# rasmusab/bayes.js

Hardware: AMD Instinct MI355X
Metric: posterior draws/sec (= param-updates/sec) (higher is better)
Workload: dtype f64

## Files before the change

bayes.js_amd/csrc/amwg_kernel.h:

```cpp
#pragma once
#if !defined(__HIPCC_RTC__)
#include <hip/hip_runtime.h>
#endif

#include "amwg_div.h"
#include "amwg_ld.h"
#include "amwg_philox.h"
#include "amwg_types.h"

namespace amwg {

struct LdsLayout {
  uint32_t data, state, pls, cnt, tot, cc, adapt, pl, idx, perm, total, stride, logpls, bc, xw;
};
__host__ __device__ inline LdsLayout lds_layout(size_t data_bytes, int P, int CPB, int max_top, int n_named, bool multi = false) {
  LdsLayout L;
  uint32_t o = 0;
  L.stride = (uint32_t)P | 1u;
  L.data = o;  o += (uint32_t)((data_bytes + 15) & ~(size_t)15);
  L.state = o; o += L.stride * CPB * 8;
  L.pls = o;   o += L.stride * CPB * 8;
  L.cnt = o;   o += L.stride * CPB * 8;
  L.tot = o;   o += (L.stride * CPB * 4 + 15) & ~15u;
  L.cc = o;    o += (uint32_t)P * sizeof(CompConst);
// ... 374 lines not shown
      "s_cselect_b64 %[m], %[OA], %[EA]\n\t"
      "s_branch 4f\n"
      "3:\n\t"
      "s_bitcmp1_b32 %[p], 0\n\t"
      "s_cselect_b64 %[m], %[OB], %[EB]\n"
      "4:\n\t"
      "s_bfe_u32 %[tmp], %[p], 0x60001\n\t"
      "s_lshr_b64 %[rest], %[m], %[tmp]\n\t"
      "s_cmp_lg_u64 %[rest], 0\n\t"
      "s_cbranch_scc1 6f\n\t"
      "s_and_b32 %[tmp], %[p], 1\n\t"
      "s_bitcmp1_b32 %[p], 7\n\t"
      "s_cbranch_scc1 5f\n\t"
      "s_or_b32 %[p], %[tmp], 0x80\n\t"
      "s_branch 2b\n"
      "5:\n\t"
      "s_or_b32 %[p], %[tmp], 0xfe\n\t"
      "s_branch 9f\n"
      "6:\n\t"
      "s_ff1_i32_b64 %[tmp], %[rest]\n\t"
      "s_lshl_b32 %[tmp], %[tmp], 1\n\t"
      "s_add_u32 %[p], %[p], %[tmp]\n\t"
      "s_mov_b32 m0, %[t]\n\t"
      "v_writelane_b32 %[ppv], %[p], m0\n\t"
      "s_add_u32 %[p], %[p], 3\n\t"
      "s_add_u32 %[t], %[t], 1\n\t"
      "s_branch 1b\n"
      "9:\n\t"
      "s_mov_b32 m0, %[km0]"
      : [p] "+s"(p), [t] "+s"(t), [ppv] "+v"(ppv), [m] "=&s"(m), [rest] "=&s"(rest), [tmp] "=&s"(tmp), [km0] "=&s"(keep_m0)
      : [EA] "s"(EA), [OA] "s"(OA), [EB] "s"(EB), [OB] "s"(OB), [top] "s"(top)
      : "scc");
#endif
}

template <int G>
__device__ __forceinline__ int chain_uniform(int v) {
#if defined(__HIP_DEVICE_COMPILE__)
  if constexpr (G >= 64) return __builtin_amdgcn_readfirstlane(v);
#endif
  return v;
}

__device__ __forceinline__ double lane_value(double v, int src) {
#if defined(__HIP_DEVICE_COMPILE__)
  const uint32_t hi = (uint32_t)__builtin_amdgcn_readlane((int)(f64_bits(v) >> 32), src);
  const uint32_t lo = (uint32_t)__builtin_amdgcn_readlane((int)(uint32_t)f64_bits(v), src);
  return bits_f64(((uint64_t)hi << 32) | (uint64_t)lo);
#else
  return v;
#endif
}

constexpr int kErrReplicasNeedOneWave = 1, kErrLaunchTooLong = 2, kErrMirrorOutOfSync = 4, kErrSweepNeedsOrderInRegisters = 8, kErrNoKernelBody = 16;
__device__ __forceinline__ void device_error(const StepArgs &a, int code) {
#if defined(__HIP_DEVICE_COMPILE__)
  if (threadIdx.x == 0) (void)atomicOr(a.ch.error, code);
#endif
}
template <class M, class = void> struct MirrorCheckOf { static constexpr bool value = false; };
template <class M> struct MirrorCheckOf<M, void_of<decltype(M::kMirrorCheck)>> { static constexpr bool value = M::kMirrorCheck; };

template <class Model, int G, int BT = 256, bool GL = false, bool SW = false, bool CT = false>
__device__ __forceinline__ void step_body(const StepArgs &a, unsigned char *smem) {
  constexpr int kPassU = SW ? (CertNeedsRows<Model>::value ? 2 : 4) : (BT >= 1024 ? 4 : 8);
  const int tid = threadIdx.x, nt = blockDim.x;
  constexpr bool kMulti = G > 64;
  if (!kMulti && a.cpb > 0 && nt != 64) { device_error(a, kErrReplicasNeedOneWave); return; }
  if (a.n_steps > 65535) { device_error(a, kErrLaunchTooLong); return; }
  const int CPB = kMulti ? G / 64 : ((a.cpb > 0 && a.cpb < nt / G) ? a.cpb : nt / G);
  const int c_raw = kMulti ? tid / 64 : tid / G;
  const int c_in = c_raw < CPB ? c_raw : CPB - 1, sub = tid % G;
  const int P = a.pl.P;
  const int n_named = a.pl.n_params;
  const LdsLayout L = lds_layout(DataBytesOf<Model, GL>::get(a.d, G, nt), P, CPB, a.pl.max_top, n_named, kMulti);

  const unsigned char *data_lds = smem + L.data;
  double *Sblk = reinterpret_cast<double *>(smem + L.state);
  CompConst *cc = reinterpret_cast<CompConst *>(smem + L.cc);
  uint8_t *adapt = smem + L.adapt;
  int32_t *pl_base = reinterpret_cast<int32_t *>(smem + L.pl), *pl_len = pl_base + n_named, *pl_top = pl_len + n_named, *pl_multidim = pl_top + n_named, *pl_inner = pl_multidim + n_named;
  const bool wide_idx = a.pl.max_top > kByteTop, wide_perm = n_named > kPackedNamed;
  const IndexColumn idx{smem + L.idx + (wide_idx ? 2 * c_in : c_in), CPB, wide_idx};
  const IndexColumn pcol{smem + L.perm + 2 * c_in, CPB, true};
  double *SDme = reinterpret_cast<double *>(smem + L.pls) + (size_t)c_in * L.stride;
  int2 *CNTme = reinterpret_cast<int2 *>(smem + L.cnt) + (size_t)c_in * L.stride;
  uint32_t *TOTme = reinterpret_cast<uint32_t *>(smem + L.tot) + (size_t)c_in * L.stride;
  double *LOGPLSme = reinterpret_cast<double *>(smem + L.logpls) + (size_t)c_in * L.stride;
  int32_t *BCme = reinterpret_cast<int32_t *>(smem + L.bc) + (size_t)c_in * L.stride;
  CrossWave xw{reinterpret_cast<double *>(smem + L.xw), 0};
  typename CacheOf<Model>::type cache = CacheOf<Model>::init();

  Model::stage(smem + L.data, a.d, tid, nt, G);
  for (int p = tid; p < P; p += nt) { cc[p] = a.cc[p]; adapt[p] = a.is_adapting[p]; }
  for (int i = tid; i < 4 * n_named; i += nt) pl_base[i] = a.pl.tab[i];
  for (int i = tid; i < n_named; i += nt) pl_inner[i] = a.pl.tab[n_named + i] / a.pl.tab[2 * n_named + i];

  const int64_t chain_raw = kMulti ? (int64_t)blockIdx.x : (int64_t)blockIdx.x * CPB + c_in;
  const bool live = chain_raw < a.C;
  const int64_t cl = live ? chain_raw : a.C - 1;
  const bool writer = live && sub == 0;
  const bool counter = sub == 0 && c_raw < CPB;
  const int64_t C = a.C;

  double *Sme = Sblk + (size_t)c_in * L.stride;
  for (int p = 0; p < P; ++p) {
    Sme[p] = a.ch.state[p * C + cl];
    SDme[p] = exp_v8(a.ch.prop_log_scale[p * C + cl]);
    CNTme[p] = make_int2(a.ch.acceptance_count[p * C + cl], a.ch.iterations_since_adaption[p * C + cl]);
    TOTme[p] = 0u;
    if constexpr (kMulti) { LOGPLSme[p] = a.ch.prop_log_scale[p * C + cl]; BCme[p] = a.ch.batch_count[p * C + cl]; }
  }
  const StateView S{Sme};
  uint64_t perm = wide_perm ? 0ull : a.ch.perm[cl];
  if (wide_perm)
    for (int k = 0; k < n_named; ++k) pcol.set(k, (int)a.ch.perm16[(int64_t)k * C + cl]);
  typename RngOf<Model, G, GL, SW>::type rng;
  if constexpr (GL) rng.init(a.seed, a.chain_offset + (uint64_t)cl, a.ch.rng_n[cl], tid, reinterpret_cast<double *>(smem + L.data + Model::gl_lds_bytes(a.d.pad, 0)) + (size_t)(tid >> 6) * 256);
  else if constexpr (SW) rng.init(a.seed, a.chain_offset + (uint64_t)cl, a.ch.rng_n[cl], tid, reinterpret_cast<double *>(smem + L.data + Model::window_offset(a.d, nt / 64)) + (size_t)(tid >> 6) * 256);
  else rng.init(a.seed, a.chain_offset + (uint64_t)cl, a.ch.rng_n[cl], tid);
  double lp_curr = a.ch.lp_curr[cl];
  __syncthreads();
  constexpr bool kCert = CT && CertifiedAt<Model, G>::value && !GL && (SW == CertNeedsRows<Model>::value);
  static_assert(kCert == CT, "a certified kernel is instantiated for a model that has no certified value at this lane count");
  constexpr bool kRefOrder = kCert && G > 1 && RefOrderOf<Model>::value;
  auto expression = [&]() -> double {
    if constexpr (kRefOrder) return Model::template reference_order<G>(cache, S, a.mc, a.d, data_lds, sub);
    else if constexpr (!GL) return log_post<Model, G, kPassU>(S, a, data_lds, sub, xw, cache);
    else return 0.0;
  };
  if constexpr (!GL) { if (a.init_lp) lp_curr = expression(); }
  double lpA = lp_curr, epsA = 0.0;
  bool lp_exact = true;
  if constexpr (kCert) { if (!a.init_lp) { epsA = a.ch.lp_eps[cl]; lp_exact = epsA == 0.0; } }
  (void)lpA; (void)epsA; (void)lp_exact;
#if defined(AMWG_AUDIT)
  constexpr bool kAudit = kCert;
#else
  constexpr bool kAudit = false;
#endif
  [[maybe_unused]] double audE = 0.0, aud_max_v = 0.0, aud_max_d = 0.0;
  [[maybe_unused]] uint32_t aud_n = 0u, aud_bad = 0u;
  [[maybe_unused]] auto audit_bin = [&](int which, double ratio) {
#if defined(AMWG_AUDIT)
    if (writer) {
      int b = 0;
      if (ratio > 0.0) { b = (int)((f64_bits(ratio) >> 52) & 0x7ffu) - 1023 + 40; b = b < 1 ? 1 : (b > 63 ? 63 : b); }
      if (!(ratio == ratio)) b = 63;
      (void)atomicAdd(cold_args()->ch.audit_hist + which * 64 + b, 1ull);
    }
#endif
  };
  [[maybe_unused]] auto audit_adversarial_u = [&](double ex, double eta, double u, int parity) -> double {
    if (!(eta < 0x1p-8) || !(ex > 0x1p-900) || !(ex < kInf)) return u;
    const double below = ex * (1.0 - 1.5 * eta), above = ex * (1.0 + 1.5 * eta);
    const double v = ((parity & 1) && above < 1.0) ? above : below;
    return (v > 0.0 && v < 1.0) ? v : u;
  };
  [[maybe_unused]] auto audit_value = [&](double A, double eps, double E) {
    if (eps == eps && eps < kInf && eps > 0.0 && E == E && __builtin_fabs(E) < kInf) {
      const double r = __builtin_fabs(A - E) / eps;
      aud_max_v = (r > aud_max_v || !(r == r)) ? r : aud_max_v;
      audit_bin(0, r);
    }
  };
  [[maybe_unused]] auto audit_difference = [&](double dA, double eta0, double dE, int verdict, double u) {
    if (eta0 == eta0 && eta0 < kInf && eta0 > 0.0 && dE == dE && __builtin_fabs(dE) < kInf) {
      const double r = __builtin_fabs(dA - dE) / eta0;
      aud_max_d = (r > aud_max_d || !(r == r)) ? r : aud_max_d;
      audit_bin(1, r);
    }
    const bool exact_acc = exp_v8(dE) > u;
    ++aud_n;
    if ((verdict > 0 && !exact_acc) || (verdict < 0 && exact_acc)) ++aud_bad;
  };
#if defined(AMWG_X_PHASES)
  uint64_t ph_acc[16];
#pragma unroll
  for (int q = 0; q < 16; ++q) ph_acc[q] = 0;
  uint64_t ph_last = __builtin_readcyclecounter();
#define AMWG_PHASE(i) do { const uint64_t ph_now = __builtin_readcyclecounter(); ph_acc[i] += ph_now - ph_last; ph_last = ph_now; } while (0)
#else
#define AMWG_PHASE(i) do { } while (0)
#endif
  auto set_state = [&](int comp, double v) {
    Sme[comp] = v;
    if constexpr (TracksState<Model>::value) Model::on_set(cache, comp, v, sub, a.d);
  };

  constexpr int D = Model::kDerived;
  const int PR = P + D;
  int64_t row = a.row0;
  int32_t next_rec = (int32_t)a.step0;
  const int P_stepped = a.pl.P_stepped;
  const bool recording = a.draws != nullptr;
  const int n_steps = a.n_steps;

  const int lane64 = tid & 63;
  int ord = lane64;
  (void)ord;
  if (SW && a.pl.max_top > 64) { device_error(a, kErrSweepNeedsOrderInRegisters); return; }
  const bool ord_in_regs = SW ? true : (G >= 64 && a.pl.max_top <= 64);
  constexpr bool kSweep = SW && !GL && LaneReuseOf<Model>::value && G == 64 && !BinaryOf<Model>::value;
  const bool sweep_rt = kSweep && ord_in_regs && a.d.pad > 0;
  if constexpr (kAudit) { if (lp_exact) audE = lp_curr; else audE = expression(); }
  wave_priority(kStepperPriority);
  auto record_draws = [&](int step) {
    if (recording && step == next_rec) {
      double *const draws = cold_args()->draws;
      {
        constexpr int LW = G < 64 ? G : 64;
        if (live && (!kMulti || sub < 64))
          for (int p = sub & (LW - 1); p < P; p += LW) {
#if !defined(AMWG_X_NOREC)
            draws[(row * PR + p) * C + cl] = S(p);
#endif
          }
      }
      if constexpr (D > 0) {
        double dv[D];
        (void)Model::template eval<G, true>(S, a.d, data_lds, sub, dv);
        if (writer)
          for (int q = 0; q < D; ++q) draws[(row * PR + P + q) * C + cl] = dv[q];
      }
      ++row;
      next_rec += cold_args()->thin;
    }
  };
  auto shuffle_named = [&]() {
    for (int i = n_named - 1; i > 0; --i) {
      const int j = (int)__builtin_floor(rng.next() * (double)(i + 1));
      if (wide_perm) { const int ti = pcol.get(i); pcol.set(i, pcol.get(j)); pcol.set(j, ti); }
      else perm = perm_swap(perm, i, j);
    }
  };
  auto adapt_component = [&](int comp, bool accepted, int2 cnt, double batch_size, bool store, bool per_lane = false) {
    cnt.x += accepted ? 1 : 0;
    cnt.y += 1;
    const bool boundary = (double)cnt.y >= batch_size;
    if (per_lane ? boundary : chain_true<GL ? 1 : G>(boundary)) {
      const CompConst k = cc[comp];
      const int64_t gi = (int64_t)comp * C + cl;
      int32_t *const g_bc = kMulti ? nullptr : cold_args()->ch.batch_count;
      double *const g_pls = kMulti ? nullptr : cold_args()->ch.prop_log_scale;
      const int32_t bc = (kMulti ? BCme[comp] : g_bc[gi]) + 1;
      const double adj = __builtin_fmin(k.max_adaptation, k.initial_adaptation / __builtin_sqrt((double)bc));
      double pls = kMulti ? LOGPLSme[comp] : g_pls[gi];
      if ((double)cnt.x / k.batch_size > k.target_accept_rate) pls += adj; else pls -= adj;
      cnt = make_int2(0, 0);
      SDme[comp] = exp_v8_cold(pls);
      if constexpr (kMulti) { BCme[comp] = bc; LOGPLSme[comp] = pls; }
      else if (store) { g_bc[gi] = bc; g_pls[gi] = pls; }
    }
    CNTme[comp] = cnt;
  };

  [[maybe_unused]] auto accept_sweep = [&](double diff, double u_accept) -> bool {
    bool accepted = false;
    if (chain_true<G>(diff >= 0.0)) accepted = true;
    else if (chain_true<G>(diff < -746.0)) accepted = false;
    else {
      const double lower = 1.0 + diff;
      if (chain_true<G>(u_accept < lower - 0x1p-50)) accepted = true;
      else if (chain_true<G>(diff > -1.0 && u_accept > (lower + 0.5 * diff * diff) + 0x1p-50)) accepted = false;
      else accepted = chain_true<G>(exp_v8(diff) > u_accept);
    }
    return chain_true<G>(accepted);
  };

#ifndef AMWG_X_GLCUT
#define AMWG_X_GLCUT 0
#endif
  if constexpr (GL) {
    static_assert(G == 64, "the group-local kernel runs a chain on one whole wavefront");
    typename Model::Lane gl;
    const int Gn = a.d.G;
    lp_curr = Model::template refresh<kPassU>(gl, S, a.mc, a.d, data_lds, lane64);
    const int comp_l = gl.grp >= 0 ? gl.grp : 0;
    const int first_of = (int)reinterpret_cast<const int8_t *>(data_lds + (size_t)a.d.pad * 64 * 8)[lane64 * 8 + 7];
    uint64_t first_mask = __ballot(gl.first);
    for (int step = 0; step < n_steps; ++step) {
      record_draws(step);
      shuffle_named();
      for (int np = 0; np < n_named; ++np) {
        const int p = __builtin_amdgcn_readfirstlane((int)perm_get(perm, np));
        const int base = __builtin_amdgcn_readfirstlane(pl_base[p]);
        if (__builtin_amdgcn_readfirstlane(pl_multidim[p]) == 0) {
          if (AMWG_X_GLCUT == 6) continue;
          const int comp = base;
          const bool is_mu = comp == Gn;
          const double cur = is_mu ? gl.mu : gl.sigma;
          const double k_lower = cc[comp].lower, k_upper = cc[comp].upper;
          const int k_type = cc[comp].type;
          const int2 cnt = CNTme[comp];
          const double batch_size = cc[comp].batch_size;
          const bool adapting = adapt[comp] != 0;
          double prop = rnorm_js(rng, cur, SDme[comp]);
          if (k_type == kTypeInt) prop = js_round(prop);
          const bool inb = !(prop < k_lower || prop > k_upper);
          bool accepted = false;
          if (inb) {
// ... 475 lines not shown
      } else if (inb) {
        double prop_lp = 0.0;
        if constexpr (kCert) {
          for (int which = chain_true<G>(lp_exact) ? 1 : 0; which < 2; ++which) {
            if (which == 0) set_state(comp, cur);
            const double v = expression();
            if (which == 0) { lp_curr = v; lp_exact = true; set_state(comp, prop); }
            else prop_lp = v;
          }
        } else {
          prop_lp = expression();
        }
#if defined(__HIP_DEVICE_COMPILE__)
        asm volatile("" : : "v"(nx.cur), "v"(nx.sd), "v"(nx.batch_size), "v"(nx.cnt.x), "v"(nx.cnt.y), "v"((int)nx.adapting));
#endif
        const double diff = prop_lp - lp_curr;
        if (chain_true<G>(diff >= 0.0)) accepted = true;
        else if (chain_true<G>(diff < -746.0)) accepted = false;
        else {
          const double lower = 1.0 + diff;
          if (chain_true<G>(u_accept < lower - 0x1p-50)) accepted = true;
          else if (chain_true<G>(diff > -1.0 && u_accept > (lower + 0.5 * diff * diff) + 0x1p-50)) accepted = false;
          else accepted = chain_true<G>(exp_v8(diff) > u_accept);
        }
        accepted = chain_true<G>(accepted);
        if (accepted) lp_curr = prop_lp;
        else set_state(comp, cur);
        if constexpr (kCert) { lpA = lp_curr; epsA = 0.0; }
        if (counter) (void)__hip_atomic_fetch_add(&TOTme[comp], 1u + (accepted ? 0x10000u : 0u), __ATOMIC_RELAXED, __HIP_MEMORY_SCOPE_WORKGROUP);
      }
      if constexpr (kAudit) { if (inb && accepted) audE = aud_E_prop; }
      AMWG_PHASE(11);
      if (chain_true<G>(me.adapting)) adapt_component(comp, accepted, me.cnt, me.batch_size, writer);
      AMWG_PHASE(12);
    }
  }

  if constexpr (kCert) {
    if (a.finalize_lp && !lp_exact) { lp_curr = expression(); lp_exact = true; }
    if (!lp_exact) lp_curr = lpA;
    if (writer) cold_args()->ch.lp_eps[cl] = lp_exact ? 0.0 : epsA;
  }
  if constexpr (!GL && MirrorCheckOf<Model>::value) {
    if (!Model::template mirror_ok<G>(cache, S, a.d, sub)) (void)atomicOr(cold_args()->ch.error, kErrMirrorOutOfSync);
  }
#if defined(AMWG_X_PHASES)
  if ((tid & 63) == 0 && live) {
    unsigned long long *const hh = cold_args()->ch.audit_hist + 64;
#pragma unroll
    for (int q = 0; q < 16; ++q) (void)atomicAdd(hh + q, (unsigned long long)ph_acc[q]);
  }
#endif
  if constexpr (kAudit) {
    if (writer) {
      double *const au = cold_args()->ch.audit;
      const double v0 = au[cl], d0 = au[C + cl];
      au[cl] = (aud_max_v > v0 || !(aud_max_v == aud_max_v)) ? aud_max_v : v0;
      au[C + cl] = (aud_max_d > d0 || !(aud_max_d == aud_max_d)) ? aud_max_d : d0;
      au[2 * C + cl] += (double)aud_n;
      au[3 * C + cl] += (double)aud_bad;
    }
  }
  if (writer) {
    const cold_args_ptr ca = cold_args();
    double *const o_state = ca->ch.state, *const o_pls = ca->ch.prop_log_scale;
    int32_t *const o_ac = ca->ch.acceptance_count, *const o_it = ca->ch.iterations_since_adaption, *const o_bc = ca->ch.batch_count;
    int32_t *const o_acc = ca->ch.accepts, *const o_inb = ca->ch.inbounds;
    for (int p = 0; p < P; ++p) {
      o_state[p * C + cl] = S(p);
      o_ac[p * C + cl] = CNTme[p].x;
      o_it[p * C + cl] = CNTme[p].y;
      o_acc[p * C + cl] += (int32_t)(TOTme[p] >> 16);
      o_inb[p * C + cl] += (int32_t)(TOTme[p] & 0xffffu);
      if constexpr (kMulti) { o_pls[p * C + cl] = LOGPLSme[p]; o_bc[p * C + cl] = BCme[p]; }
    }
    if (wide_perm) { uint16_t *const o_p16 = ca->ch.perm16; for (int k = 0; k < n_named; ++k) o_p16[(int64_t)k * C + cl] = (uint16_t)pcol.get(k); }
    else ca->ch.perm[cl] = perm;
    ca->ch.rng_n[cl] = rng.consumed();
    ca->ch.lp_curr[cl] = lp_curr;
  }
}

template <class M, class = void> struct MinWavesOf { static constexpr int value = 1; };
template <class M> struct MinWavesOf<M, void_of<decltype(M::kMinWavesPerSimd)>> { static constexpr int value = M::kMinWavesPerSimd; };

template <class Model, int G, int BT>
__global__ void __launch_bounds__(BT, MinWavesOf<Model>::value) amwg_step_kernel(const StepArgs a) {
  extern __shared__ __attribute__((aligned(16))) unsigned char smem[];
  step_body<Model, G, BT>(a, smem);
}
template <class Model, int BT>
__global__ void __launch_bounds__(BT, MinWavesOf<Model>::value) amwg_sweep_kernel(const StepArgs a) {
  extern __shared__ __attribute__((aligned(16))) unsigned char smem[];
  step_body<Model, 64, BT, false, true>(a, smem);
}
template <class Model, int G, int BT>
__global__ void __launch_bounds__(BT, MinWavesOf<Model>::value) amwg_step_kernel_cert(const StepArgs a) {
  extern __shared__ __attribute__((aligned(16))) unsigned char smem[];
  step_body<Model, G, BT, false, false, true>(a, smem);
}
template <class Model, int BT>
__global__ void __launch_bounds__(BT, MinWavesOf<Model>::value) amwg_sweep_kernel_cert(const StepArgs a) {
  extern __shared__ __attribute__((aligned(16))) unsigned char smem[];
  step_body<Model, 64, BT, false, true, true>(a, smem);
}
template <class Model, int BT>
__global__ void __launch_bounds__(BT, MinWavesOf<Model>::value) amwg_gl_kernel(const StepArgs a) {
  extern __shared__ __attribute__((aligned(16))) unsigned char smem[];
  step_body<Model, 64, BT, true>(a, smem);
}

}
```

bayes.js_amd/csrc/amwg_kernels.hip:

```cpp
#include <hip/hip_runtime.h>

#include <type_traits>

#include "amwg_dataset.h"
#include "amwg_host.h"
#include "amwg_kernel.h"
#include "amwg_models.h"

using namespace amwg;

#if AMWG_FAMILY == 0
using Family = NormalModel;
#elif AMWG_FAMILY == 1
using Family = BetaBernModel;
#elif AMWG_FAMILY == 2
using Family = HierNormalModel;
#elif AMWG_FAMILY == 3
using Family = PoisGlmModel;
#else
#error "AMWG_FAMILY must be 0..3"
#endif

namespace {

#if defined(AMWG_X_BT1024)
constexpr int class_of(int) { return 1024; }
#else
constexpr int class_of(int block) { return block <= 256 ? 256 : (block <= 512 ? 512 : 1024); }
#endif

constexpr bool kHasTwin = !std::is_same_v<Family, HierNormalModel>;
template <int G, int BT>
KernelPair step_pair() {
  if constexpr (kHasTwin) return {amwg_step_kernel<Family, G, BT>, amwg_step_kernel_ds<Family, G, BT>};
  else return {amwg_step_kernel<Family, G, BT>, nullptr};
}

template <int G>
KernelPair single_wave(int block) {
  switch (class_of(block)) {
    case 256: return step_pair<G, 256>();
    case 512: if constexpr (Family::kMaxThreads >= 512) return step_pair<G, 512>(); else return {};
    default: if constexpr (Family::kMaxThreads >= 1024) return step_pair<G, 1024>(); else return {};
  }
}
template <int G>
KernelPair multi_wave(int block) {
  if (block != G) return {};
  if constexpr (G <= Family::kMaxThreads) return step_pair<G, class_of(G)>();
  else return {};
}

}

#if AMWG_FAMILY == 2
step_kernel_t amwg_kernel_hier_gl(int block) {
  switch (class_of(block)) {
    case 256: return amwg_gl_kernel<HierGlModel, 256>;
    case 512: return amwg_gl_kernel<HierGlModel, 512>;
    default: return amwg_gl_kernel<HierGlModel, 1024>;
// ... 60 lines not shown
```

bayes.js_amd/csrc/amwg_models.h:

```cpp
#pragma once
#include "amwg_div.h"
#include "amwg_ld.h"
#include "amwg_pass.h"
#include "amwg_twoval.h"
#include "amwg_types.h"
#include "amwg_window.h"

namespace amwg {

__device__ __forceinline__ double norm_const_sd(double v, double m, double c_sd, double den, double y_hi, double y_lo, int den_ok) {
  const double t = v - m;
  const double tt = t * t;
  const double q = (den_ok && wide_range(tt)) ? div_by_invariant(tt, den, Reciprocal{y_hi, y_lo}) : tt / den;
  return c_sd - q;
}

struct NormCache {
  double sd, c, den;
  Reciprocal y;
  bool den_ok;
};
__device__ __forceinline__ NormCache norm_cache_init() { return NormCache{__builtin_nan(""), 0.0, 0.0, Reciprocal{0.0, 0.0}, false}; }
AMWG_HD NormCache norm_cache_make(double sd, double neg_half_log_2pi) {
  NormCache k;
// ... 49 lines not shown
    lp += (sigma < mc.ua || sigma > mc.ub) ? -kInf : mc.lunif;
    return lp;
  }
  static constexpr bool kTracksState = true;
  struct Cache { NormCache n; double mu, sigma; bool loaded; };
  __device__ __forceinline__ static Cache cache_init() { return Cache{norm_cache_init(), 0.0, 0.0, false}; }
  __device__ __forceinline__ static void on_set(Cache &k, int comp, double v, int, const DataRef &) { k.mu = comp == 0 ? v : k.mu; k.sigma = comp == 0 ? k.sigma : v; }
  static constexpr bool kMirrorCheck = true;
  template <int GL>
  __device__ __forceinline__ static bool mirror_ok(const Cache &k, const StateView &S, const DataRef &, int) {
    return !k.loaded || (f64_bits(k.mu) == f64_bits(S(0)) && f64_bits(k.sigma) == f64_bits(S(1)));
  }
  template <int GL>
  __device__ __forceinline__ static void load(Cache &k, const StateView &S, const ModelConsts &, const DataRef &, const unsigned char *, int) {
    if (!k.loaded) { k.mu = S(0); k.sigma = S(1); k.loaded = true; }
  }
  template <int GL>
  __device__ __forceinline__ static Pass begin(const StateView &, const ModelConsts &mc, const DataRef &d,
                                               const unsigned char *smem, Cache &kc) {
    Pass ps;
    NormCache &k = kc.n;
    ps.mu = kc.mu;
    norm_cache_update(k, kc.sigma, mc.neg_half_log_2pi);
    ps.c = k.c;
    ps.den = k.den;
    ps.y = k.y;
    ps.fast = !mc.exact_division && mc.data_mid_range && k.den_ok &&
              (ps.mu == 0 || mid_range(__builtin_fabs(ps.mu)));
    ps.x = GL == 1 ? d.x : reinterpret_cast<const double *>(smem);
    return ps;
  }
  template <bool FAST>
  __device__ __forceinline__ static double term(const Pass &ps, int i) {
    const double t = ps.x[i] - ps.mu;
    const double tt = t * t;
    return ps.c - (FAST ? div_by_invariant(tt, ps.den, ps.y) : tt / ps.den);
  }
  template <int G>
  __device__ inline __attribute__((noinline)) static double pass_slow_impl(const double *x, double mu, double c, double den, int n_obs, int sub, double acc) {
    for (int i = sub; i < n_obs; i += G) { const double t = x[i] - mu; acc += c - (t * t) / den; }
    return acc;
  }
  template <int G>
  __device__ __forceinline__ static double pass_slow(const Pass &ps, int n_obs, int sub, double acc) { return pass_slow_impl<G>(ps.x, ps.mu, ps.c, ps.den, n_obs, sub, acc); }
  static constexpr bool kStagedFast = true;
  template <int G, int U = 8>
  __device__ __forceinline__ static double pass_fast(const Pass &ps, int n_obs, int sub, double acc) {
    if constexpr (G == 1) return norm_pass_uniform<8>(ps.x, ps.mu, ps.c, ps.den, ps.y, n_obs, acc);
    else return norm_pass_staged<G, U, false>(ps.x, nullptr, StateView{nullptr}, ps.mu, ps.c, ps.den, ps.y, n_obs, sub, acc);
  }
  static constexpr bool kCertified = true;
  static constexpr int kCertifiedLanes = 1;
  struct Approx { double value, eps; };
  template <int G, int BT>
  __device__ __forceinline__ static Approx log_post_approx(Cache &kc, const StateView &S, const ModelConsts &mc, const DataRef &d, const unsigned char *smem, int sub) {
    static_assert(G == 1, "the certified pass of the Normal family is the one-lane one");
    load<G>(kc, S, mc, d, smem, sub);
    norm_cache_update(kc.n, kc.sigma, mc.neg_half_log_2pi);
    const double P = prior(S, mc, d, kc);
    double S2;
    if (mc.sufficient) {
      const double dm = (mc.suff_xbar_hi - kc.mu) + mc.suff_xbar_lo;
      S2 = __builtin_fma((double)d.n_obs, dm * dm, mc.suff_ss);
    } else
    if constexpr (BT <= 512) {
      constexpr int B = BT <= 256 ? kWaveBlock : 8;
      double *scr = wave_scratch_of(d);
      const bool tile = lds_bytes_of(d, 1, 0) != 0;
      if (tile && scr != nullptr) S2 = norm_sq_pass_wave<B, true>((amwg_lds_f64_ptr)smem, kc.mu, d.n_obs, scr);
      else S2 = norm_sq_pass_wave<B>(tile ? reinterpret_cast<const double *>(smem) : d.x, kc.mu, d.n_obs, scr);
    }
    else S2 = norm_sq_pass_uniform<8>(d.x, kc.mu, d.n_obs);
    const double n = (double)d.n_obs;
    const double Q = S2 * kc.n.y.hi, nc = n * kc.n.c;
    const double mag = __builtin_fabs(P) + __builtin_fabs(nc) + 2.0 * Q;
    return Approx{(P + nc) - Q, (2.0 * n + 64.0) * 0x1p-53 * mag * 1.25};
  }
};

struct BetaBernModel {
  static constexpr bool kSplitPrior = false;
  static constexpr bool kUser = false, kHasFast = false, kOneLanePass = true;
  static constexpr int kDerived = 0;
  static constexpr bool kHasBinary = false;
  static constexpr int kMaxThreads = 1024;
  static constexpr int kUnroll = 8;
  struct Pass { double l1, l0; const uint8_t *x; const uint32_t *bits; bool has_invalid, fast_forward; BitData B; };
  __host__ __device__ static size_t words(int n_obs) { return (size_t)n_obs / 32 + 2; }
  static constexpr size_t kFfLdsLimit = 120 * 1024;
  __host__ __device__ static size_t lds_bytes(int n_obs, int, int lanes) {
    if (lanes == 1) { const size_t b = 6 * words(n_obs) * 4; return b <= kFfLdsLimit ? ((b + 15) & ~(size_t)15) : 0; }
    return ((size_t)n_obs + 15) & ~(size_t)15;
  }
  __device__ static void stage(unsigned char *smem, const DataRef &d, int tid, int nt, int lanes) {
    if (lanes == 1) {
      if (lds_bytes(d.n_obs, 0, 1) == 0) return;
      uint32_t *dst = reinterpret_cast<uint32_t *>(smem);
      const uint32_t *src = static_cast<const uint32_t *>(d.arr[0]);
      for (int k = tid; k < (int)(6 * words(d.n_obs)); k += nt) dst[k] = src[k];
      return;
    }
    for (int i = tid; i < d.n_obs; i += nt) smem[i] = d.xb[i];
  }
  template <class C>
  __device__ __forceinline__ static double prior(const StateView &S, const ModelConsts &mc, const DataRef &, C &) {
    const double th = S(0);
    double lp = 0;
    if (th > 1 || th < 0) lp += -kInf;
    else if (mc.ba == 1 && mc.bb == 1) lp += 0.0;
    else lp += (mc.ba - 1) * log_v8(th) + (mc.bb - 1) * log_v8(1 - th) - mc.lbeta_ab;
    return lp;
  }
  struct Cache {};
  __device__ __forceinline__ static Cache cache_init() { return Cache{}; }
  template <int GL>
  __device__ __forceinline__ static Pass begin(const StateView &S, const ModelConsts &mc, const DataRef &d,
                                               const unsigned char *smem, Cache &) {
    Pass ps;
    const double th = S(0);
    ps.l1 = log_v8(th);
    ps.l0 = log_v8(1 - th);
    ps.x = smem;
    ps.bits = d.xw;
    ps.has_invalid = mc.has_invalid != 0;
    ps.fast_forward = !mc.exact_division;
    {
      const size_t W = words(d.n_obs);
      const uint32_t *base = lds_bytes(d.n_obs, 0, 1) ? reinterpret_cast<const uint32_t *>(smem) : static_cast<const uint32_t *>(d.arr[0]);
      ps.B.w = base; ps.B.pre = base + W; ps.B.om1 = base + 2 * W; ps.B.po1 = base + 3 * W; ps.B.om0 = base + 4 * W; ps.B.po0 = base + 5 * W;
      ps.B.n = d.n_obs;
// ... 829 lines not shown
```

bayes.js_amd/csrc/amwg_run.hip:

```cpp
#include <dlfcn.h>
#include <sys/mman.h>

#include <cmath>
#include <cstddef>
#include <cstdlib>
#include <mutex>
#include <unordered_map>

#include "../../include/amwg_selftest.h"
#include "amwg_autocov.h"
#include "amwg_covariance.h"
#include "amwg_fold.h"
#include "amwg_histogram.h"
#include "amwg_host.h"
#include "amwg_kernel.h"
#include "amwg_dataset.h"
#include "amwg_user_dataset.h"

using namespace amwg;

int use_device(int device) {
  int ndev = 0;
  hipError_t e = hipGetDeviceCount(&ndev);
  if (e != hipSuccess || ndev < 1) return amwg_fail(AMWG_EHIP, "no HIP device available (%s)", hipGetErrorString(e));
// ... 100 lines not shown
    } else if (s->n_datasets > 1) {
      hipLaunchKernelGGL(s->ds_kernel, dim3(p.grid), dim3(p.block), (size_t)p.lds, s->stream, a, ds);
      HIP_TRY(hipGetLastError());
    } else {
      hipLaunchKernelGGL(s->kernel, dim3(p.grid), dim3(p.block), (size_t)p.lds, s->stream, a);
      HIP_TRY(hipGetLastError());
    }
    s->lp_ready = true;
    if (finalize || a.init_lp) s->lp_is_expression = true;
    if (m > 0 && !finalize && info(p.variant).certified) s->lp_is_expression = false;
    if (!quiet) s->n_launches++;
    if (d_draws) row += (m > a.step0) ? (m - a.step0 + thin - 1) / thin : 0;
    const int64_t marked = s->chunk_rows.empty() ? 0 : s->chunk_rows.back();
    if (!win && d_draws && d_draws == s->d_draws && row > marked &&
        (done + m >= n || (double)(row - marked) * (double)(s->P + s->D) * (double)s->C * 8.0 >= 8388608.0)) {
      const size_t j = s->chunk_rows.size();
      if (j >= s->chunk_ev.size()) {
        hipEvent_t e = nullptr;
        HIP_TRY(hipEventCreateWithFlags(&e, hipEventDisableTiming));
        s->chunk_ev.push_back(e);
      }
      HIP_TRY(hipEventRecord(s->chunk_ev[j], s->stream));
      s->chunk_rows.push_back(row);
    }
    done += m;
    if (win && row > 0 && (row == win->window_rows || done >= n)) {
      if (row > win->window_rows || folded + row > win->total_rows) return amwg_fail(AMWG_EINVAL, "internal: %lld rows in a window of %lld (%lld of %lld folded)", (long long)row, (long long)win->window_rows, (long long)folded, (long long)win->total_rows);
      if (win->cov)
        TRYB(amwg_comoment_window(d_draws, folded, row, s->P + s->D, s->C, win->cov->d_values, win->cov->n_values, win->acc, win->cov->d_co, s->stream));
      TRYB(amwg_fold_window(d_draws, folded, row, win->total_rows / 2, s->P + s->D, s->C, win->acc, s->stream));
      if (win->hist)
        TRYB(amwg_histogram_launch("amwg_sample_summarize", d_draws, row, s->P + s->D, s->C, s->n_datasets, win->hist->d_edges, win->hist->bins, win->hist->uniform, win->hist->d_counts, s->stream));
      if (win->acf)
        TRYB(amwg_autocov_window(d_draws, folded, row, s->P + s->D, s->C, win->acf->d_values, win->acf->n_values, win->acf->max_lag, win->acf->d_state, s->stream));
      win->windows++;
      folded += row;
      row = 0;
    }
  } while (done < n);
  if (!quiet) HIP_TRY(hipEventRecord(s->ev1, s->stream));
  return AMWG_OK;
}

int finish_timing(amwg_sampler *s) {
  HIP_TRY(hipEventSynchronize(s->ev1));
  float ms = 0;
  HIP_TRY(hipEventElapsedTime(&ms, s->ev0, s->ev1));
  s->kernel_ms = ms;
  if (s->ch.error) {
    int32_t bits = 0;
    HIP_TRY(hipMemcpy(&bits, s->ch.error, sizeof bits, hipMemcpyDeviceToHost));
    if (bits) {
      HIP_TRY(hipMemset(s->ch.error, 0, sizeof bits));
      return amwg_fail(AMWG_EHIP, "the step kernel reported an internal error (bits %d:%s%s%s%s%s): the chains' state is not to be trusted", bits,
                       (bits & kErrReplicasNeedOneWave) ? " replicated chains in a workgroup of more than one wavefront" : "",
                       (bits & kErrLaunchTooLong) ? " more than 65535 steps in one launch" : "",
                       (bits & kErrMirrorOutOfSync) ? " the register mirror of the state is out of sync with the state" : "",
                       (bits & kErrSweepNeedsOrderInRegisters) ? " the sweep kernel was launched for a parameter vector of more than 64 entries" : "",
                       (bits & kErrNoKernelBody) ? " the launched kernel has no body for this closure at this geometry" : "");
    }
  }
  return AMWG_OK;
}

#ifndef MADV_POPULATE_WRITE
#define MADV_POPULATE_WRITE 23
#endif
static void prefault(char *p, size_t bytes) {
  if (!p || !bytes) return;
  const size_t page = 4096;
  const uintptr_t a0 = ((uintptr_t)p + page - 1) & ~(uintptr_t)(page - 1), a1 = ((uintptr_t)p + bytes) & ~(uintptr_t)(page - 1);
  if (a1 > a0 && madvise(reinterpret_cast<void *>(a0), a1 - a0, MADV_POPULATE_WRITE) == 0) {
    volatile char *q = p;
    q[0] = q[0];
    q[bytes - 1] = q[bytes - 1];
    return;
  }
  volatile char *q = p;
  for (size_t o = 0; o < bytes; o += page) q[o] = q[o];
  q[bytes - 1] = q[bytes - 1];
}
Prefaulter::Prefaulter(size_t n_chunks) : done(n_chunks), per_chunk(n_chunks, 0) { for (auto &d : done) d.store(0); }
void Prefaulter::add(char *p, size_t bytes, size_t chunk) {
  const size_t step = (size_t)8 << 20;
  for (size_t o = 0; o < bytes; o += step) { pieces.push_back({p + o, bytes - o < step ? bytes - o : step, chunk}); per_chunk[chunk]++; }
}
void Prefaulter::start(int n_threads) {
  for (int t = 0; t < n_threads; ++t)
    workers.emplace_back([this] {
      for (;;) {
        const size_t i = next.fetch_add(1);
        if (i >= pieces.size()) return;
        prefault(pieces[i].p, pieces[i].bytes);
        done[pieces[i].chunk].fetch_add(1, std::memory_order_release);
      }
    });
}
void Prefaulter::wait_chunk(size_t j) {
  while (done[j].load(std::memory_order_acquire) < per_chunk[j]) {
    const size_t i = next.fetch_add(1);
    if (i < pieces.size()) { prefault(pieces[i].p, pieces[i].bytes); done[pieces[i].chunk].fetch_add(1, std::memory_order_release); }
    else std::this_thread::yield();
  }
}
Prefaulter::~Prefaulter() { for (auto &w : workers) w.join(); }

namespace {
std::mutex g_summaries_mu;
std::unordered_map<const amwg_sampler *, FoldSummary> g_summaries;
FoldSummary &summary_slot(const amwg_sampler *s) {
  std::lock_guard<std::mutex> lock(g_summaries_mu);
  return g_summaries[s];
// ... 249 lines not shown
```

Baseline: 1.496 billion.

## Add specialized lean one-lane certified stepper for the two-parameter Normal model

Adds a dedicated kernel body for the Normal model at one lane per chain, used in the certified kernel. It keeps the two parameters, proposal scales and counters in scalar registers instead of the generic LDS-backed state arrays, and drops the generic permutation and adaptation machinery. It also raises the wave block size for the data pass from the default to 16 rows. The cost is a second code path that must stay in sync with the generic one, guarded by a shape check that reports a new device error.

```diff
diff --git a/bayes.js_amd/csrc/amwg_kernel.h b/bayes.js_amd/csrc/amwg_kernel.h
--- a/bayes.js_amd/csrc/amwg_kernel.h
+++ b/bayes.js_amd/csrc/amwg_kernel.h
@@ -450,12 +450,55 @@
 #endif
 }
 
-constexpr int kErrReplicasNeedOneWave = 1, kErrLaunchTooLong = 2, kErrMirrorOutOfSync = 4, kErrSweepNeedsOrderInRegisters = 8, kErrNoKernelBody = 16;
+constexpr int kErrReplicasNeedOneWave = 1, kErrLaunchTooLong = 2, kErrMirrorOutOfSync = 4, kErrSweepNeedsOrderInRegisters = 8, kErrNoKernelBody = 16, kErrLeanShape = 32;
 __device__ __forceinline__ void device_error(const StepArgs &a, int code) {
 #if defined(__HIP_DEVICE_COMPILE__)
   if (threadIdx.x == 0) (void)atomicOr(a.ch.error, code);
 #endif
 }
+struct AdaptedScale { int32_t batch_count; double prop_log_scale; };
+__device__ __forceinline__ AdaptedScale adapt_scale(const CompConst &k, int32_t batch_count, double prop_log_scale, int32_t acceptance_count) {
+  const int32_t bc = batch_count + 1;
+  const double adj = __builtin_fmin(k.max_adaptation, k.initial_adaptation / __builtin_sqrt((double)bc));
+  double pls = prop_log_scale;
+  if ((double)acceptance_count / k.batch_size > k.target_accept_rate) pls += adj; else pls -= adj;
+  return AdaptedScale{bc, pls};
+}
+
+__device__ __forceinline__ void audit_count_bin([[maybe_unused]] const ChainArrays &ch, [[maybe_unused]] bool writer, [[maybe_unused]] int which, [[maybe_unused]] double ratio) {
+#if defined(AMWG_AUDIT)
+  if (writer) {
+    int b = 0;
+    if (ratio > 0.0) { b = (int)((f64_bits(ratio) >> 52) & 0x7ffu) - 1023 + 40; b = b < 1 ? 1 : (b > 63 ? 63 : b); }
+    if (!(ratio == ratio)) b = 63;
+    (void)atomicAdd(ch.audit_hist + which * 64 + b, 1ull);
+  }
+#endif
+}
+__device__ __forceinline__ double audit_place_u(double ex, double eta, double u, int parity) {
+  if (!(eta < 0x1p-8) || !(ex > 0x1p-900) || !(ex < kInf)) return u;
+  const double below = ex * (1.0 - 1.5 * eta), above = ex * (1.0 + 1.5 * eta);
+  const double v = ((parity & 1) && above < 1.0) ? above : below;
+  return (v > 0.0 && v < 1.0) ? v : u;
+}
+__device__ __forceinline__ double audit_ratio(double A, double eps, double E) {
+  if (eps == eps && eps < kInf && eps > 0.0 && E == E && __builtin_fabs(E) < kInf) return __builtin_fabs(A - E) / eps;
+  return -1.0;
+}
+__device__ __forceinline__ void audit_max(double &m, double r) { m = (r > m || !(r == r)) ? r : m; }
+__device__ __forceinline__ void audit_verdict(uint32_t &n, uint32_t &bad, double dE, int verdict, double u) {
+  const bool exact_acc = exp_v8(dE) > u;
+  ++n;
+  if ((verdict > 0 && !exact_acc) || (verdict < 0 && exact_acc)) ++bad;
+}
+__device__ __forceinline__ void audit_store(double *au, int64_t C, int64_t cl, double max_v, double max_d, uint32_t n, uint32_t bad) {
+  const double v0 = au[cl], d0 = au[C + cl];
+  au[cl] = (max_v > v0 || !(max_v == max_v)) ? max_v : v0;
+  au[C + cl] = (max_d > d0 || !(max_d == max_d)) ? max_d : d0;
+  au[2 * C + cl] += (double)n;
+  au[3 * C + cl] += (double)bad;
+}
+
 template <class M, class = void> struct MirrorCheckOf { static constexpr bool value = false; };
 template <class M> struct MirrorCheckOf<M, void_of<decltype(M::kMirrorCheck)>> { static constexpr bool value = M::kMirrorCheck; };
 
@@ -539,38 +582,16 @@
 #endif
   [[maybe_unused]] double audE = 0.0, aud_max_v = 0.0, aud_max_d = 0.0;
   [[maybe_unused]] uint32_t aud_n = 0u, aud_bad = 0u;
-  [[maybe_unused]] auto audit_bin = [&](int which, double ratio) {
-#if defined(AMWG_AUDIT)
-    if (writer) {
-      int b = 0;
-      if (ratio > 0.0) { b = (int)((f64_bits(ratio) >> 52) & 0x7ffu) - 1023 + 40; b = b < 1 ? 1 : (b > 63 ? 63 : b); }
-      if (!(ratio == ratio)) b = 63;
-      (void)atomicAdd(cold_args()->ch.audit_hist + which * 64 + b, 1ull);
-    }
-#endif
-  };
-  [[maybe_unused]] auto audit_adversarial_u = [&](double ex, double eta, double u, int parity) -> double {
-    if (!(eta < 0x1p-8) || !(ex > 0x1p-900) || !(ex < kInf)) return u;
-    const double below = ex * (1.0 - 1.5 * eta), above = ex * (1.0 + 1.5 * eta);
-    const double v = ((parity & 1) && above < 1.0) ? above : below;
-    return (v > 0.0 && v < 1.0) ? v : u;
-  };
+  [[maybe_unused]] auto audit_bin = [&](int which, double ratio) { audit_count_bin(cold_args()->ch, writer, which, ratio); };
+  [[maybe_unused]] auto audit_adversarial_u = [&](double ex, double eta, double u, int parity) -> double { return audit_place_u(ex, eta, u, parity); };
   [[maybe_unused]] auto audit_value = [&](double A, double eps, double E) {
-    if (eps == eps && eps < kInf && eps > 0.0 && E == E && __builtin_fabs(E) < kInf) {
-      const double r = __builtin_fabs(A - E) / eps;
-      aud_max_v = (r > aud_max_v || !(r == r)) ? r : aud_max_v;
-      audit_bin(0, r);
-    }
+    const double r = audit_ratio(A, eps, E);
+    if (!(r < 0.0)) { audit_max(aud_max_v, r); audit_bin(0, r); }
   };
   [[maybe_unused]] auto audit_difference = [&](double dA, double eta0, double dE, int verdict, double u) {
-    if (eta0 == eta0 && eta0 < kInf && eta0 > 0.0 && dE == dE && __builtin_fabs(dE) < kInf) {
-      const double r = __builtin_fabs(dA - dE) / eta0;
-      aud_max_d = (r > aud_max_d || !(r == r)) ? r : aud_max_d;
-      audit_bin(1, r);
-    }
-    const bool exact_acc = exp_v8(dE) > u;
-    ++aud_n;
-    if ((verdict > 0 && !exact_acc) || (verdict < 0 && exact_acc)) ++aud_bad;
+    const double r = audit_ratio(dA, eta0, dE);
+    if (!(r < 0.0)) { audit_max(aud_max_d, r); audit_bin(1, r); }
+    audit_verdict(aud_n, aud_bad, dE, verdict, u);
   };
 #if defined(AMWG_X_PHASES)
   uint64_t ph_acc[16];
@@ -641,10 +662,9 @@
       const int64_t gi = (int64_t)comp * C + cl;
       int32_t *const g_bc = kMulti ? nullptr : cold_args()->ch.batch_count;
       double *const g_pls = kMulti ? nullptr : cold_args()->ch.prop_log_scale;
-      const int32_t bc = (kMulti ? BCme[comp] : g_bc[gi]) + 1;
-      const double adj = __builtin_fmin(k.max_adaptation, k.initial_adaptation / __builtin_sqrt((double)bc));
-      double pls = kMulti ? LOGPLSme[comp] : g_pls[gi];
-      if ((double)cnt.x / k.batch_size > k.target_accept_rate) pls += adj; else pls -= adj;
+      const AdaptedScale ad = adapt_scale(k, kMulti ? BCme[comp] : g_bc[gi], kMulti ? LOGPLSme[comp] : g_pls[gi], cnt.x);
+      const int32_t bc = ad.batch_count;
+      const double pls = ad.prop_log_scale;
       cnt = make_int2(0, 0);
       SDme[comp] = exp_v8_cold(pls);
       if constexpr (kMulti) { BCme[comp] = bc; LOGPLSme[comp] = pls; }
@@ -1226,14 +1246,7 @@
   }
 #endif
   if constexpr (kAudit) {
-    if (writer) {
-      double *const au = cold_args()->ch.audit;
-      const double v0 = au[cl], d0 = au[C + cl];
-      au[cl] = (aud_max_v > v0 || !(aud_max_v == aud_max_v)) ? aud_max_v : v0;
-      au[C + cl] = (aud_max_d > d0 || !(aud_max_d == aud_max_d)) ? aud_max_d : d0;
-      au[2 * C + cl] += (double)aud_n;
-      au[3 * C + cl] += (double)aud_bad;
-    }
+    if (writer) audit_store(cold_args()->ch.audit, C, cl, aud_max_v, aud_max_d, aud_n, aud_bad);
   }
   if (writer) {
     const cold_args_ptr ca = cold_args();
@@ -1268,10 +1281,13 @@
   extern __shared__ __attribute__((aligned(16))) unsigned char smem[];
   step_body<Model, 64, BT, false, true>(a, smem);
 }
+template <class M, class = void> struct LeanOneLaneOf { static constexpr bool value = false; };
+template <class M> struct LeanOneLaneOf<M, void_of<decltype(M::kLeanOneLane)>> { static constexpr bool value = M::kLeanOneLane; };
 template <class Model, int G, int BT>
 __global__ void __launch_bounds__(BT, MinWavesOf<Model>::value) amwg_step_kernel_cert(const StepArgs a) {
   extern __shared__ __attribute__((aligned(16))) unsigned char smem[];
-  step_body<Model, G, BT, false, false, true>(a, smem);
+  if constexpr (G == 1 && LeanOneLaneOf<Model>::value) Model::template lean_one_lane<BT>(a, smem);
+  else step_body<Model, G, BT, false, false, true>(a, smem);
 }
 template <class Model, int BT>
 __global__ void __launch_bounds__(BT, MinWavesOf<Model>::value) amwg_sweep_kernel_cert(const StepArgs a) {
diff --git a/bayes.js_amd/csrc/amwg_kernels.hip b/bayes.js_amd/csrc/amwg_kernels.hip
--- a/bayes.js_amd/csrc/amwg_kernels.hip
+++ b/bayes.js_amd/csrc/amwg_kernels.hip
@@ -6,6 +6,7 @@
 #include "amwg_host.h"
 #include "amwg_kernel.h"
 #include "amwg_models.h"
+#include "amwg_normal1.h"
 
 using namespace amwg;
 
diff --git a/bayes.js_amd/csrc/amwg_models.h b/bayes.js_amd/csrc/amwg_models.h
--- a/bayes.js_amd/csrc/amwg_models.h
+++ b/bayes.js_amd/csrc/amwg_models.h
@@ -125,7 +125,7 @@
   static constexpr bool kCertified = true;
   static constexpr int kCertifiedLanes = 1;
   struct Approx { double value, eps; };
-  template <int G, int BT>
+  template <int G, int BT, int WB = (BT <= 256 ? kWaveBlock : 8)>
   __device__ __forceinline__ static Approx log_post_approx(Cache &kc, const StateView &S, const ModelConsts &mc, const DataRef &d, const unsigned char *smem, int sub) {
     static_assert(G == 1, "the certified pass of the Normal family is the one-lane one");
     load<G>(kc, S, mc, d, smem, sub);
@@ -137,7 +137,7 @@
       S2 = __builtin_fma((double)d.n_obs, dm * dm, mc.suff_ss);
     } else
     if constexpr (BT <= 512) {
-      constexpr int B = BT <= 256 ? kWaveBlock : 8;
+      constexpr int B = WB;
       double *scr = wave_scratch_of(d);
       const bool tile = lds_bytes_of(d, 1, 0) != 0;
       if (tile && scr != nullptr) S2 = norm_sq_pass_wave<B, true>((amwg_lds_f64_ptr)smem, kc.mu, d.n_obs, scr);
@@ -149,6 +149,9 @@
     const double mag = __builtin_fabs(P) + __builtin_fabs(nc) + 2.0 * Q;
     return Approx{(P + nc) - Q, (2.0 * n + 64.0) * 0x1p-53 * mag * 1.25};
   }
+  static constexpr bool kLeanOneLane = true;
+  template <int BT>
+  __device__ __forceinline__ static void lean_one_lane(const StepArgs &a, unsigned char *smem);
 };
 
 struct BetaBernModel {
diff --git a/bayes.js_amd/csrc/amwg_normal1.h b/bayes.js_amd/csrc/amwg_normal1.h
--- /dev/null
+++ b/bayes.js_amd/csrc/amwg_normal1.h
@@ -0,0 +1,222 @@
+#pragma once
+#include "amwg_kernel.h"
+#include "amwg_models.h"
+
+namespace amwg {
+
+#ifndef AMWG_LEAN_WAVE_BLOCK
+#define AMWG_LEAN_WAVE_BLOCK 16
+#endif
+constexpr int kLeanWaveBlock = AMWG_LEAN_WAVE_BLOCK;
+
+template <int BT>
+__device__ __forceinline__ void normal_one_lane_body(const StepArgs &a, unsigned char *smem) {
+  using Model = NormalModel;
+  constexpr int G = 1;
+  constexpr int kPassU = BT >= 1024 ? 4 : 8;
+  constexpr int kRows = BT <= 256 ? kLeanWaveBlock : 8;
+  const int tid = threadIdx.x, nt = blockDim.x;
+  {
+    const int32_t *const t = a.pl.tab;
+    bool ok = a.pl.P == 2 && a.pl.n_params == 2 && a.pl.P_stepped == 2 && a.cpb == 0;
+    if (ok) ok = t[0] == 0 && t[1] == 1 && t[2] == 1 && t[3] == 1 && t[6] == 0 && t[7] == 0 && (a.cc[0].type == kTypeReal || a.cc[0].type == kTypeInt) && (a.cc[1].type == kTypeReal || a.cc[1].type == kTypeInt);
+    if (!ok) { device_error(a, kErrLeanShape); return; }
+  }
+  if (a.n_steps > 65535) { device_error(a, kErrLaunchTooLong); return; }
+  const unsigned char *data_lds = smem;
+  Model::stage(smem, a.d, tid, nt, G);
+
+  const int64_t chain_raw = (int64_t)blockIdx.x * nt + tid;
+  const int64_t C = a.C;
+  const bool live = chain_raw < C;
+  const int64_t cl = live ? chain_raw : C - 1;
+  const bool writer = live;
+
+  const double lower0 = a.cc[0].lower, upper0 = a.cc[0].upper, bsize0 = a.cc[0].batch_size;
+  const double lower1 = a.cc[1].lower, upper1 = a.cc[1].upper, bsize1 = a.cc[1].batch_size;
+  const bool int0 = a.cc[0].type == kTypeInt, int1 = a.cc[1].type == kTypeInt;
+  const bool adapting0 = a.is_adapting[0] != 0, adapting1 = a.is_adapting[1] != 0;
+
+  Model::Cache cache = Model::cache_init();
+  cache.mu = a.ch.state[cl];
+  cache.sigma = a.ch.state[C + cl];
+  cache.loaded = true;
+  const StateView S{nullptr};
+  double sd0 = exp_v8(a.ch.prop_log_scale[cl]), sd1 = exp_v8(a.ch.prop_log_scale[C + cl]);
+  int2 cnt0 = make_int2(a.ch.acceptance_count[cl], a.ch.iterations_since_adaption[cl]);
+  int2 cnt1 = make_int2(a.ch.acceptance_count[C + cl], a.ch.iterations_since_adaption[C + cl]);
+  uint32_t tot0 = 0u, tot1 = 0u;
+  uint64_t perm = a.ch.perm[cl];
+  CoopStream<G> rng;
+  rng.init(a.seed, a.chain_offset + (uint64_t)cl, a.ch.rng_n[cl], tid);
+  double lp_curr = a.ch.lp_curr[cl];
+  __syncthreads();
+
+  CrossWave xw{nullptr, 0};
+  auto expression = [&]() -> double { return log_post<Model, G, kPassU>(S, a, data_lds, 0, xw, cache); };
+  auto set_state = [&](int comp, double v) { Model::on_set(cache, comp, v, 0, a.d); };
+  if (a.init_lp) lp_curr = expression();
+  double lpA = lp_curr, epsA = 0.0;
+  bool lp_exact = true;
+  if (!a.init_lp) { epsA = a.ch.lp_eps[cl]; lp_exact = epsA == 0.0; }
+#if defined(AMWG_AUDIT)
+  constexpr bool kAudit = true;
+#else
+  constexpr bool kAudit = false;
+#endif
+  [[maybe_unused]] double audE = 0.0, aud_max_v = 0.0, aud_max_d = 0.0;
+  [[maybe_unused]] uint32_t aud_n = 0u, aud_bad = 0u;
+#if defined(AMWG_X_PHASES)
+  uint64_t ph_acc[16];
+#pragma unroll
+  for (int q = 0; q < 16; ++q) ph_acc[q] = 0;
+  uint64_t ph_last = __builtin_readcyclecounter();
+#endif
+  int64_t row = a.row0;
+  int32_t next_rec = (int32_t)a.step0;
+  const bool recording = a.draws != nullptr;
+  const int n_steps = a.n_steps;
+  if constexpr (kAudit) { if (lp_exact) audE = lp_curr; else audE = expression(); }
+  wave_priority(kStepperPriority);
+
+  for (int step = 0; step < n_steps; ++step) {
+    AMWG_PHASE(15);
+    if (recording && step == next_rec) {
+      double *const draws = cold_args()->draws;
+      if (live) {
+#if !defined(AMWG_X_NOREC)
+        draws[(row * 2 + 0) * C + cl] = cache.mu;
+        draws[(row * 2 + 1) * C + cl] = cache.sigma;
+#endif
+      }
+      ++row;
+      next_rec += cold_args()->thin;
+    }
+    {
+      const int j = (int)__builtin_floor(rng.next() * 2.0);
+      perm = perm_swap(perm, 1, j);
+    }
+    AMWG_PHASE(0);
+    AMWG_PHASE(1);
+#pragma unroll 1
+    for (int slot = 0; slot < 2; ++slot) {
+      const int comp = (int)perm_get(perm, slot);
+      const bool first = comp == 0;
+      AMWG_PHASE(14);
+      const double cur = first ? cache.mu : cache.sigma;
+      const int2 cnt = first ? cnt0 : cnt1;
+      double prop = rnorm_js(rng, cur, first ? sd0 : sd1);
+      if (first ? int0 : int1) prop = js_round(prop);
+      const bool inb = !(prop < (first ? lower0 : lower1) || prop > (first ? upper0 : upper1));
+      double u_accept = 0.0;
+      if (inb) { set_state(comp, prop); u_accept = rng.next(); }
+      AMWG_PHASE(8);
+      AMWG_PHASE(9);
+      bool accepted = false, certified = false;
+      [[maybe_unused]] double aud_E_prop = 0.0;
+      if (__ballot(inb) != 0ull) {
+        wave_priority(0);
+        const Model::Approx r = Model::template log_post_approx<G, BT, kRows>(cache, S, a.mc, a.d, data_lds, 0);
+        wave_priority(kStepperPriority);
+        AMWG_PHASE(10);
+        if (inb) {
+          const double dA = r.value - lpA;
+          const double eta = ((r.eps + epsA + __builtin_fabs(dA) * 0x1p-51) * 1.0625 + 0x1p-49) * a.bound_scale;
+          const double ex = exp_v8(dA);
+          if constexpr (kAudit) { if (a.audit_adversarial) u_accept = audit_place_u(ex, eta, u_accept, step + slot); }
+          const int verdict = certified_test(dA, eta, ex, u_accept);
+          if constexpr (kAudit) {
+            aud_E_prop = expression();
+            const ChainArrays &ch = cold_args()->ch;
+            const double rv = audit_ratio(r.value, r.eps, aud_E_prop);
+            if (!(rv < 0.0)) { audit_max(aud_max_v, rv); audit_count_bin(ch, writer, 0, rv); }
+            const double dE = aud_E_prop - audE;
+            const double rd = audit_ratio(dA, (r.eps + epsA + __builtin_fabs(dA) * 0x1p-51) * 1.0625, dE);
+            if (!(rd < 0.0)) { audit_max(aud_max_d, rd); audit_count_bin(ch, writer, 1, rd); }
+            audit_verdict(aud_n, aud_bad, dE, verdict, u_accept);
+          }
+          if (verdict > 0) { certified = true; accepted = true; lpA = r.value; epsA = r.eps; lp_exact = false; }
+          else if (verdict < 0) { certified = true; set_state(comp, cur); }
+        }
+      }
+      if (!certified && inb) {
+        double prop_lp = 0.0;
+        for (int which = lp_exact ? 1 : 0; which < 2; ++which) {
+          if (which == 0) set_state(comp, cur);
+          const double v = expression();
+          if (which == 0) { lp_curr = v; lp_exact = true; set_state(comp, prop); }
+          else prop_lp = v;
+        }
+        const double diff = prop_lp - lp_curr;
+        if (diff >= 0.0) accepted = true;
+        else if (diff < -746.0) accepted = false;
+        else {
+          const double lower = 1.0 + diff;
+          if (u_accept < lower - 0x1p-50) accepted = true;
+          else if (diff > -1.0 && u_accept > (lower + 0.5 * diff * diff) + 0x1p-50) accepted = false;
+          else accepted = exp_v8(diff) > u_accept;
+        }
+        if (accepted) lp_curr = prop_lp;
+        else set_state(comp, cur);
+        lpA = lp_curr; epsA = 0.0;
+      }
+      if (inb) { const uint32_t t = 1u + (accepted ? 0x10000u : 0u); tot0 += first ? t : 0u; tot1 += first ? 0u : t; }
+      if constexpr (kAudit) { if (inb && accepted) audE = aud_E_prop; }
+      AMWG_PHASE(11);
+      if (first ? adapting0 : adapting1) {
+        int2 c = cnt;
+        c.x += accepted ? 1 : 0;
+        c.y += 1;
+        if ((double)c.y >= (first ? bsize0 : bsize1)) {
+          const cold_args_ptr ca = cold_args();
+          const CompConst k = ca->cc[comp];
+          const int64_t gi = (int64_t)comp * C + cl;
+          int32_t *const g_bc = ca->ch.batch_count;
+          double *const g_pls = ca->ch.prop_log_scale;
+          const AdaptedScale ad = adapt_scale(k, g_bc[gi], g_pls[gi], c.x);
+          c = make_int2(0, 0);
+          const double sd = exp_v8_cold(ad.prop_log_scale);
+          sd0 = first ? sd : sd0;
+          sd1 = first ? sd1 : sd;
+          if (writer) { g_bc[gi] = ad.batch_count; g_pls[gi] = ad.prop_log_scale; }
+        }
+        cnt0 = first ? c : cnt0;
+        cnt1 = first ? cnt1 : c;
+      }
+      AMWG_PHASE(12);
+    }
+  }
+
+  if (a.finalize_lp && !lp_exact) { lp_curr = expression(); lp_exact = true; }
+  if (!lp_exact) lp_curr = lpA;
+#if defined(AMWG_X_PHASES)
+  if ((tid & 63) == 0 && live) {
+    unsigned long long *const hh = cold_args()->ch.audit_hist + 64;
+#pragma unroll
+    for (int q = 0; q < 16; ++q) (void)atomicAdd(hh + q, (unsigned long long)ph_acc[q]);
+  }
+#endif
+  if constexpr (kAudit) { if (writer) audit_store(cold_args()->ch.audit, C, cl, aud_max_v, aud_max_d, aud_n, aud_bad); }
+  if (writer) {
+    const cold_args_ptr ca = cold_args();
+    ca->ch.lp_eps[cl] = lp_exact ? 0.0 : epsA;
+    ca->ch.state[cl] = cache.mu;
+    ca->ch.state[C + cl] = cache.sigma;
+    ca->ch.acceptance_count[cl] = cnt0.x;
+    ca->ch.acceptance_count[C + cl] = cnt1.x;
+    ca->ch.iterations_since_adaption[cl] = cnt0.y;
+    ca->ch.iterations_since_adaption[C + cl] = cnt1.y;
+    ca->ch.accepts[cl] += (int32_t)(tot0 >> 16);
+    ca->ch.accepts[C + cl] += (int32_t)(tot1 >> 16);
+    ca->ch.inbounds[cl] += (int32_t)(tot0 & 0xffffu);
+    ca->ch.inbounds[C + cl] += (int32_t)(tot1 & 0xffffu);
+    ca->ch.perm[cl] = perm;
+    ca->ch.rng_n[cl] = rng.consumed();
+    ca->ch.lp_curr[cl] = lp_curr;
+  }
+}
+
+template <int BT>
+__device__ __forceinline__ void NormalModel::lean_one_lane(const StepArgs &a, unsigned char *smem) { normal_one_lane_body<BT>(a, smem); }
+
+}
diff --git a/bayes.js_amd/csrc/amwg_run.hip b/bayes.js_amd/csrc/amwg_run.hip
--- a/bayes.js_amd/csrc/amwg_run.hip
+++ b/bayes.js_amd/csrc/amwg_run.hip
@@ -176,12 +176,13 @@
     HIP_TRY(hipMemcpy(&bits, s->ch.error, sizeof bits, hipMemcpyDeviceToHost));
     if (bits) {
       HIP_TRY(hipMemset(s->ch.error, 0, sizeof bits));
-      return amwg_fail(AMWG_EHIP, "the step kernel reported an internal error (bits %d:%s%s%s%s%s): the chains' state is not to be trusted", bits,
+      return amwg_fail(AMWG_EHIP, "the step kernel reported an internal error (bits %d:%s%s%s%s%s%s): the chains' state is not to be trusted", bits,
                        (bits & kErrReplicasNeedOneWave) ? " replicated chains in a workgroup of more than one wavefront" : "",
                        (bits & kErrLaunchTooLong) ? " more than 65535 steps in one launch" : "",
                        (bits & kErrMirrorOutOfSync) ? " the register mirror of the state is out of sync with the state" : "",
                        (bits & kErrSweepNeedsOrderInRegisters) ? " the sweep kernel was launched for a parameter vector of more than 64 entries" : "",
-                       (bits & kErrNoKernelBody) ? " the launched kernel has no body for this closure at this geometry" : "");
+                       (bits & kErrNoKernelBody) ? " the launched kernel has no body for this closure at this geometry" : "",
+                       (bits & kErrLeanShape) ? " the Normal family's one-lane stepper was launched for something other than two scalar parameters of real or int type" : "");
     }
   }
   return AMWG_OK;
```

Result: faster. 1.527 billion, median of 6 (+2.1%).
